# ArjunTeh/AdjointNonlinearRayTracing

Measured on AMD Instinct MI355X. Metric: ray-steps/sec (fwd+adjoint), 256^3 RIF grid, 1M rays x 512 steps, higher is better.
Workload: dtype f32

## Files before the change

adjointnonlinearraytracing_amd/_lib.py:

```python
from __future__ import annotations

import ctypes as C
import os
from typing import Optional

_HERE = os.path.dirname(os.path.abspath(__file__))
LIB_PATH = os.environ.get("DRRT_HIP_LIB") or os.path.join(_HERE, "libdrrt_hip.so")

FLAG_NONE = 0
FLAG_SORT_RAYS = 1
FLAG_CORRECTED_H = 2
FLAG_NO_ZERO = 4
FLAG_DIRECT_ATOMICS = 8
FLAG_DEBUG_COUNTERS = 16
FLAG_PAIR_GRID = 64
FLAG_PAIR_REUSE = 128
FLAG_QUAD_GRID, FLAG_QUAD_REUSE = FLAG_PAIR_GRID, FLAG_PAIR_REUSE
FLAG_Q16_POS_ONLY = 0x200000
FLAG_STATIC_WINDOW = 0x400000
FLAG_CHORD_KEY = 0x800000
FLAG_RING_WINDOW = 0x1000000
FLAG_DISPATCH_IN_ORDER = 0x2000000
FLAG_RING_SPARSE, FLAG_RING_GENERAL, FLAG_RING_DIRECT = 0x4000000, 0x8000000, 0x10000000
ADAM_MASK_BOUNDARY, ADAM_CLAMP_MIN = 1, 2

ERR_RES_MISMATCH, ERR_BAD_RES, ERR_ARG, ERR_HIP = -1, -2, -3, -4


class Stats(C.Structure):
    _fields_ = [("ray_steps", C.c_ulonglong), ("n_failed", C.c_ulonglong),
                ("iters", C.c_uint), ("reserved", C.c_uint)]


STATS_BYTES = C.sizeof(Stats)

_vp, _f, _sz, _u, _ll, _i = C.c_void_p, C.c_float, C.c_size_t, C.c_uint, C.c_longlong, C.c_int
_d = C.c_double
_tail = [_vp, _vp, _sz, _u, _vp]

SIGNATURES = {
    "drrt_workspace_bytes": (_sz, [_sz, _u]),
    "drrt_workspace_bytes_grid": (_sz, [_sz, _ll, _u]),
    "drrt_last_error": (C.c_char_p, []),
    "drrt_version": (C.c_char_p, []),
    "drrt_trace_f32": (_i, [_vp, _ll, _vp, _sz, _vp, _vp, _f, _f, _vp, _vp] + _tail),
    "drrt_trace_f16io": (_i, [_vp, _ll, _vp, _sz, _vp, _vp, _f, _f, _vp, _vp] + _tail),
# ... 19 lines not shown
    "drrt_backtrace_sdf_rays_f32": (_i, [_vp, _vp, _ll, _vp, _sz, _vp, _vp, _vp, _vp, _f, _f, _vp, _vp] + _tail),
    "drrt_sensor_splat_f32": (_i, [_sz, _vp, _vp, _vp, _f, _vp, _vp, _vp, _vp, _i, _f, _vp, _u, _vp]),
    "drrt_sensor_splat_bwd_f32": (_i, [_sz, _vp, _vp, _vp, _f, _vp, _vp, _vp, _vp, _i, _f, _vp, _vp, _vp, _vp]),
    "drrt_sensor_far_splat_f32": (_i, [_sz, _vp, _vp, _f, _vp, _vp, _i, _f, _vp, _u, _vp]),
    "drrt_sensor_far_splat_bwd_f32": (_i, [_sz, _vp, _vp, _f, _vp, _vp, _i, _f, _vp, _vp, _vp, _vp]),
    "drrt_sensor_tex_get_f32": (_i, [_sz, _vp, _vp, _vp, _vp, _vp, _vp, _vp, _i, _f, _i, _vp, _vp]),
    "drrt_sensor_tex_get_bwd_f32": (_i, [_sz, _vp, _vp, _vp, _vp, _vp, _vp, _vp, _i, _f, _i, _vp, _vp, _vp, _vp]),
    "drrt_sensor_splat_dframe_f32": (_i, [_sz, _vp, _vp, _vp, _f, _vp, _i, _f, _vp, _u, _vp]),
    "drrt_sensor_splat_dframe_bwd_f32": (_i, [_sz, _vp, _vp, _vp, _f, _vp, _i, _f, _vp, _vp, _vp, _vp]),
    "drrt_sensor_far_splat_dframe_f32": (_i, [_sz, _vp, _vp, _f, _vp, _i, _f, _vp, _u, _vp]),
    "drrt_sensor_far_splat_dframe_bwd_f32": (_i, [_sz, _vp, _vp, _f, _vp, _i, _f, _vp, _vp, _vp, _vp]),
    "drrt_sensor_tex_get_dframe_f32": (_i, [_sz, _vp, _vp, _vp, _vp, _i, _f, _i, _vp, _vp]),
    "drrt_sensor_tex_get_dframe_bwd_f32": (_i, [_sz, _vp, _vp, _vp, _vp, _i, _f, _i, _vp, _vp, _vp, _vp]),
    "drrt_rays_to_plane_f32": (_i, [_sz, _vp, _vp, _vp, _vp, _i, _vp, _vp]),
    "drrt_rays_to_plane_bwd_f32": (_i, [_sz, _vp, _vp, _vp, _vp, _i, _vp, _vp, _vp, _vp]),
    "drrt_upres_volume_f32": (_i, [_vp, _vp, _vp, _vp, _vp]),
    "drrt_adam_step_f32": (_i, [_vp, _vp, _vp, _vp, _vp, _d, _d, _d, _d, _d, _d, _d, _u, _vp]),
    "drrt_gen_workspace_bytes": (_sz, [_i, _i, _i, _i]),
    "drrt_gen_rays_f32": (_i, [_i, _vp, _vp, _i, _i, _i, _i, _d, _d, _i, _i, _vp, _d, _vp, _vp, _vp, _vp, _vp, _sz, _vp]),
    "drrt_gen_cone_rays_f32": (_i, [_vp, _vp, _i, _i, _i, _i, _d, _d, _d, _vp, _d, _vp, _vp, _vp, _vp, _vp, _sz, _vp]),
    "drrt_last_order": (_vp, [_vp]),
    "drrt_set_order_hint": (None, [_vp, _sz]),
    "drrt_order_hint_pending": (_sz, []),
    "drrt_last_steps": (_vp, [_vp]),
    "drrt_set_step_hint": (None, [_vp, _sz]),
    "drrt_last_bundle_counters": (_vp, []),
    "drrt_ring_threshold_pct": (_i, []),
    "drrt_ring_long_threshold_permille": (_i, []),
    "drrt_ring_direct_threshold_pct": (_i, []),
    "drrt_profile_begin": (_i, [_i]),
    "drrt_profile_collect": (_i, [_vp, _vp, _i]),
    "drrt_profile_end": (None, []),
}

PROF_NAMES = {1: "trace", 2: "backtrace", 3: "sort", 4: "zero", 5: "quad", 6: "backtrace_rays",
              7: "backtrace_cable_rays", 8: "backtrace_pln_rays", 9: "backtrace_sdf_rays"}

_lib: Optional[C.CDLL] = None


def load() -> C.CDLL:
    global _lib
    if _lib is not None:
        return _lib
    if not os.path.exists(LIB_PATH):
        raise RuntimeError(
# ... 27 lines not shown
```

adjointnonlinearraytracing_amd/csrc/drrt_api.hip:

```cpp
#include "drrt_march.h"

using namespace drrt;

namespace drrt {
size_t sort_workspace_bytes(size_t n);
hipError_t sort_rays_by_entry_voxel(const Vol& V, float h, size_t n, const void* pos, const void* vel, int io_half,
                                    float dir_sign, void* ws, size_t ws_bytes, const uint32_t** perm_out,
                                    hipStream_t stream, bool chord_key);
}

static thread_local char g_err[512] = "";

static int fail(int code, const char* msg) {
  snprintf(g_err, sizeof(g_err), "%s", msg);
  return code;
}
static int fail_hip(hipError_t e, const char* where) {
  snprintf(g_err, sizeof(g_err), "%s: %s", where, hipGetErrorString(e));
  return DRRT_ERR_HIP;
}

namespace drrt { int sensor_fail(int code, const char* msg) { return fail(code, msg); } }

extern "C" const char* drrt_last_error(void) { return g_err; }

static thread_local const uint32_t* g_last_order = nullptr;
static thread_local size_t g_last_order_n = 0;
static thread_local const uint32_t* g_hint_order = nullptr;
static thread_local size_t g_hint_n = 0;

static thread_local const uint32_t* g_last_steps = nullptr;
// ... 4 lines not shown
static inline OrderHint take_hint() {
  OrderHint h{g_hint_order, g_hint_n, g_hint_steps, g_hint_steps_n};
  g_hint_order = nullptr; g_hint_n = 0;
  g_hint_steps = nullptr; g_hint_steps_n = 0;
  return h;
}

extern "C" const uint32_t* drrt_last_order(size_t* n_out) {
  if (n_out) *n_out = g_last_order_n;
  return g_last_order;
}
extern "C" void drrt_set_order_hint(const uint32_t* order, size_t n) { g_hint_order = order; g_hint_n = order ? n : 0; }
extern "C" size_t drrt_order_hint_pending(void) { return g_hint_order ? g_hint_n : (g_hint_steps ? g_hint_steps_n : 0); }
extern "C" const uint32_t* drrt_last_steps(size_t* n_out) {
  if (n_out) *n_out = g_last_steps_n;
  return g_last_steps;
}
extern "C" void drrt_set_step_hint(const uint32_t* steps, size_t n) { g_hint_steps = steps; g_hint_steps_n = steps ? n : 0; }
static thread_local const unsigned* g_last_counters = nullptr;
extern "C" const unsigned* drrt_last_bundle_counters(void) { return g_last_counters; }
extern "C" int drrt_ring_threshold_pct(void) { return DRRT_RING_MIN_NOFIT_PCT; }
extern "C" int drrt_ring_long_threshold_permille(void) { return DRRT_RING_MIN_LONG_PERMILLE; }
extern "C" int drrt_ring_direct_threshold_pct(void) { return DRRT_RING_DIRECT_MAX_PAIR_PCT; }

struct ProfRec { hipEvent_t a, b; int id; };
static ProfRec* g_prof = nullptr;
static int g_prof_cap = 0, g_prof_n = 0;

struct ProfScope {
  int slot; hipStream_t s;
  ProfScope(int id, hipStream_t st) : slot(-1), s(st) {
    if (g_prof && g_prof_n < g_prof_cap) {
      slot = g_prof_n++;
      g_prof[slot].id = id;
      (void)hipEventRecord(g_prof[slot].a, s);
    }
  }
  ~ProfScope() { if (slot >= 0) (void)hipEventRecord(g_prof[slot].b, s); }
};

extern "C" void drrt_profile_end(void) {
  for (int i = 0; i < g_prof_cap; ++i) { (void)hipEventDestroy(g_prof[i].a); (void)hipEventDestroy(g_prof[i].b); }
  delete[] g_prof; g_prof = nullptr; g_prof_cap = g_prof_n = 0;
}

extern "C" int drrt_profile_begin(int capacity) {
// ... 83 lines not shown
  if (nvox >= (1LL << 29)) return fail(DRRT_ERR_ARG, "grid too large (>= 2^29 voxels) for 32-bit byte offsets");
  if (res[0] >= (1 << 24) || res[1] >= (1 << 24) || res[2] >= (1 << 24) || (long long)res[0] * res[1] >= (1 << 24))
    return fail(DRRT_ERR_ARG, "grid extents too large for 24-bit index arithmetic");
  if (!(h > 0.f) || !(h < 3.0e38f)) return fail(DRRT_ERR_ARG, "h and ds must be positive and finite");
  V->data = rif; V->W = res[0]; V->H = res[1]; V->D = res[2];
  vol_finish(*V, h);
  return DRRT_OK;
}

static inline int max3(const int r[3]) { return r[0] > r[1] ? (r[0] > r[2] ? r[0] : r[2]) : (r[1] > r[2] ? r[1] : r[2]); }

static inline int steps_fwd(float h, const int res[3], float ds)  { return (int)(4.0f * h * (float)max3(res) / ds); }
static inline int steps_sdf(float h, const int res[3], float ds)  { return (int)(2.0f * h * (float)max3(res) / ds); }
static inline int steps_adj(float h, const int res[3], float ds)  { return (int)(2.0f * h * (float)max3(res) / ds); }

static int zero_stats(drrt_stats* stats, hipStream_t s) {
  if (!stats) return DRRT_OK;
  hipError_t e = hipMemsetAsync(stats, 0, sizeof(drrt_stats), s);
  return e == hipSuccess ? DRRT_OK : fail_hip(e, "hipMemsetAsync(stats)");
}

static int maybe_sort(const Vol& V, float h, size_t n, const void* pos, const void* vel, float dir_sign,
                      unsigned flags, void* ws, size_t ws_bytes, const uint32_t** perm, hipStream_t s,
                      OrderHint hint, int io_half = 0) {
  *perm = nullptr;
  if (hint.order && hint.n == n) { *perm = hint.order; return DRRT_OK; }
  if (!(flags & DRRT_FLAG_SORT_RAYS) || n < 2) return DRRT_OK;
  if (!ws || ws_bytes < sort_workspace_bytes(n)) return fail(DRRT_ERR_ARG, "workspace too small for DRRT_FLAG_SORT_RAYS");
  ProfScope prof(DRRT_PROF_SORT, s);
  hipError_t e = sort_rays_by_entry_voxel(V, h, n, pos, vel, io_half, dir_sign, ws, ws_bytes, perm, s,
                                          (flags & DRRT_FLAG_CHORD_KEY) != 0);
  if (e == hipSuccess) { g_last_order = *perm; g_last_order_n = n; }
  return e == hipSuccess ? DRRT_OK : fail_hip(e, "sort_rays_by_entry_voxel");
}

#define LAUNCH_CHECK(where)                                              \
  do { hipError_t e_ = hipGetLastError(); if (e_ != hipSuccess) return fail_hip(e_, where); } while (0)

static int private_stats(drrt_stats** stats) {
  constexpr int kMaxDev = 64;
  static drrt_stats* priv[kMaxDev] = {};
  int dev = 0;
  hipError_t e = hipGetDevice(&dev);
  if (e != hipSuccess) return fail_hip(e, "hipGetDevice");
  if (dev < 0 || dev >= kMaxDev) return fail(DRRT_ERR_ARG, "device ordinal out of range; pass a stats block");
  if (!priv[dev]) { e = hipMalloc((void**)&priv[dev], sizeof(drrt_stats)); if (e != hipSuccess) return fail_hip(e, "hipMalloc(stats)"); }
  *stats = priv[dev];
  return DRRT_OK;
}

template <int MODE>
static int run_trace(const float* rif, const float* sdf, long long nvox, const int res[3], size_t n,
                     const void* pos, const void* vel, const float* pln_o, const float* pln_d,
                     float h, float ds, void* xt, void* vt, uint8_t* failmask, drrt_stats* stats,
                     void* ws, size_t ws_bytes, unsigned flags, void* stream, int io_half = 0) {
  const OrderHint hint = take_hint();
  g_err[0] = 0;
  hipStream_t s = (hipStream_t)stream;
  TraceArgs a{};
  int rc = make_vol(rif, nvox, res, h, &a.vol); if (rc) return rc;
  rc = check_steps(h, ds); if (rc) return rc;
  if (n == 0) return zero_stats(stats, s);
  if (!pos || !vel || !xt || !vt) return fail(DRRT_ERR_ARG, "null ray pointer");
  if (MODE == 1 && (!pln_o || !pln_d || !failmask)) return fail(DRRT_ERR_ARG, "null plane/failmask pointer");
  if ((MODE == 1 || MODE == 2) && !stats) { rc = private_stats(&stats); if (rc) return rc; }
  if (MODE == 2 && !sdf) return fail(DRRT_ERR_ARG, "null sdf pointer");
  if (n > 0xffffffffULL) return fail(DRRT_ERR_ARG, "too many rays for uint32 permutation");
  rc = zero_stats(stats, s); if (rc) return rc;
  rc = maybe_sort(a.vol, h, n, pos, vel, 1.f, flags, ws, ws_bytes, &a.perm, s, hint, io_half); if (rc) return rc;
  rc = maybe_pair(a.vol, nvox, n, flags, ws, ws_bytes, s); if (rc) return rc;
  if (MODE == 2) {
    const size_t off = (flags & DRRT_FLAG_SORT_RAYS) ? align_up(sort_workspace_bytes(n), 256) : 0;
    if (!ws || ws_bytes < off + n) return fail(DRRT_ERR_ARG, "workspace too small for trace_sdf (see drrt_workspace_bytes)");
    a.again = (uint8_t*)ws + off;
  }
  g_last_steps = nullptr; g_last_steps_n = 0;
  if (MODE != 2) {
    const size_t off = (flags & DRRT_FLAG_SORT_RAYS) ? align_up(sort_workspace_bytes(n), 256) : 0;
    if (ws && ws_bytes >= off + n * sizeof(uint32_t)) {
      a.steps_out = (uint32_t*)((char*)ws + off);
      g_last_steps = a.steps_out; g_last_steps_n = n;
    }
  }
  a.io_half = io_half;
  a.sdf = sdf; a.pos = pos; a.vel = vel; a.pln_o = pln_o; a.pln_d = pln_d;
  a.xt = xt; a.vt = vt; a.failmask = failmask; a.stats = stats; a.n = n; a.ds = ds;
  a.max_steps = (MODE == 2) ? steps_sdf(h, res, ds) : steps_fwd(h, res, ds);
  a.xcd_order = (a.perm != nullptr && !(flags & DRRT_FLAG_DISPATCH_IN_ORDER)) ? 1 : 0;
  {
    ProfScope prof(DRRT_PROF_TRACE, s);
    launch_trace(MODE, a, s);
  }
// ... 115 lines not shown
  if (n == 0) return zero_stats(stats, s);
  if (!pos || !vel || !target || !xt || !vt || !dist2) return fail(DRRT_ERR_ARG, "null ray pointer");
  if (n > 0xffffffffULL) return fail(DRRT_ERR_ARG, "too many rays for uint32 permutation");
  if (!stats) return fail(DRRT_ERR_ARG, "trace_target needs a stats block (global loop count)");
  const size_t state_bytes = align_up(n * 7 * sizeof(float), 256);
  const size_t sort_bytes = (flags & DRRT_FLAG_SORT_RAYS) ? align_up(sort_workspace_bytes(n), 256) : 0;
  if (!ws || ws_bytes < state_bytes + sort_bytes) return fail(DRRT_ERR_ARG, "workspace too small for trace_target");
  rc = zero_stats(stats, s); if (rc) return rc;
  a.state = (float*)ws;
  rc = maybe_sort(a.vol, h, n, pos, vel, 1.f, flags, (char*)ws + state_bytes, ws_bytes - state_bytes, &a.perm, s,
                  OrderHint{nullptr, 0, nullptr, 0});
  if (rc) return rc;
  a.pos = pos; a.vel = vel; a.target = target; a.xt = xt; a.vt = vt; a.dist2 = dist2;
  a.stats = stats; a.n = n; a.ds = ds; a.max_steps = steps_fwd(h, res, ds);
  rc = maybe_pair(a.vol, nvox, n, flags, ws, ws_bytes, s); if (rc) return rc;
  launch_target(a, s);
  LAUNCH_CHECK("k_target");
  return DRRT_OK;
}

struct ChunkReq { void* state; size_t state_bytes; int it_begin, it_count; int* progress; };

namespace drrt {
__global__ void k_chunk_progress_init(int* p) {
  const int k = threadIdx.x;
  if (k < 20) p[k] = (k == 12 || k == 19) ? 0 : ((((k < 12 ? k : k - 1) / 3) & 1) ? (int)0x80000000 : 0x7fffffff);
}
}

struct BackPlan {
  bool direct = false;
  bool classify = false;
  bool ring_general = false;
  int ring_sparse = -1;
  bool box = false;
};
static BackPlan plan_backtrace(int mode, unsigned flags, bool chunk, bool dbg, bool classifiable) {
  BackPlan p;
  if (flags & DRRT_FLAG_DIRECT_ATOMICS) { p.direct = true; return p; }
  if ((flags & DRRT_FLAG_RING_WINDOW) && !chunk) {
    if ((flags & DRRT_FLAG_RING_SPARSE) && mode == 0 && !dbg) p.ring_sparse = (flags & DRRT_FLAG_RING_DIRECT) ? 1 : 0;
    else p.ring_general = true;
    return p;
  }
  p.box = true;
  if ((flags & DRRT_FLAG_STATIC_WINDOW) || chunk || !classifiable) return p;
// ... 13 lines not shown
  g_err[0] = 0;
  hipStream_t s = (hipStream_t)stream;
  BackArgs a{};
  int rc = make_vol(rif, nvox, res, h, &a.vol); if (rc) return rc;
  rc = check_steps(h, ds); if (rc) return rc;
  if (!grad) return fail(DRRT_ERR_ARG, "null grad pointer");
  if (MODE == 1 && !sdf) return fail(DRRT_ERR_ARG, "null sdf pointer");
  const unsigned ablation = (flags >> 8) & 0xffu;
  if (ablation > 1u) return fail(DRRT_ERR_ARG, "flags: bits 8..15 must be 0, or 1 (no adjoint launch)");
  const bool first_chunk = ck == nullptr || ck->it_begin == 0;
  if (ck != nullptr) {
    if (ck->it_begin < 0) return fail(DRRT_ERR_ARG, "chunk: it_begin must be >= 0");
    if (flags & DRRT_FLAG_DIRECT_ATOMICS) return fail(DRRT_ERR_ARG, "chunk: not available with DRRT_FLAG_DIRECT_ATOMICS");
    if (!ck->state || ck->state_bytes < drrt_backtrace_chunk_state_bytes(n))
      return fail(DRRT_ERR_ARG, "chunk: state buffer too small (see drrt_backtrace_chunk_state_bytes)");
    if (!first_chunk && (flags & DRRT_FLAG_SORT_RAYS) && !(hint.order && hint.n == n))
      return fail(DRRT_ERR_ARG, "chunk: a resumed chunk needs the visit order of its first chunk (drrt_set_order_hint)");
  }
  if (!(flags & DRRT_FLAG_NO_ZERO) && first_chunk) {
    ProfScope prof(DRRT_PROF_ZERO, s);
    hipError_t e = hipMemsetAsync(grad, 0, (size_t)nvox * sizeof(float), s);
    if (e != hipSuccess) return fail_hip(e, "hipMemsetAsync(grad)");
  }
  if (first_chunk) { rc = zero_stats(stats, s); if (rc) return rc; }
  if (n == 0) return DRRT_OK;
  if (!xt || !vt || !dx || !dv) return fail(DRRT_ERR_ARG, "null ray pointer");
  if (n > 0xffffffffULL) return fail(DRRT_ERR_ARG, "too many rays for uint32 permutation");
  if (ablation == 1u) return DRRT_OK;
  rc = maybe_sort(a.vol, h, n, xt, vt, -1.f, flags, ws, ws_bytes, &a.perm, s, hint, io_half); if (rc) return rc;
  rc = maybe_pair(a.vol, nvox, n, flags, ws, ws_bytes, s); if (rc) return rc;
  a.io_half = io_half;
  a.sdf = sdf; a.xt = xt; a.vt = vt; a.dx = dx; a.dv = dv; a.grad = grad; a.stats = stats;
  a.n = n; a.ds = ds; a.max_steps = steps_adj(h, res, ds);
  if (ck != nullptr) {
    const int left = a.max_steps - ck->it_begin;
    a.max_steps = ck->it_count < 0 ? left : (ck->it_count < left ? ck->it_count : left);
    if (a.max_steps < 0) a.max_steps = 0;
    a.chunk_state = (float*)ck->state; a.chunk_stride = (size_t)adj_grid_for(n) * kAdjBlock;
    a.chunk_resume = first_chunk ? 0 : 1; a.chunk_progress = ck->progress;
    if (ck->progress) { hipLaunchKernelGGL(drrt::k_chunk_progress_init, dim3(1), dim3(64), 0, s, ck->progress); LAUNCH_CHECK("k_chunk_progress_init"); }
  }
  a.grad_scale = (flags & DRRT_FLAG_CORRECTED_H) ? a.vol.inv_h : 1.0f;
  a.fsteps = (hint.steps && hint.steps_n == n) ? hint.steps : nullptr;
  a.xcd_order = (a.perm != nullptr && !(flags & DRRT_FLAG_DISPATCH_IN_ORDER)) ? 1 : 0;
  a.dbg = nullptr;
  if (flags & DRRT_FLAG_DEBUG_COUNTERS) {
    if (!ws || ws_bytes < 512) return fail(DRRT_ERR_ARG, "workspace too small for DRRT_FLAG_DEBUG_COUNTERS");
    a.dbg = (unsigned long long*)((char*)ws + ((ws_bytes - 512) & ~(size_t)7));
    hipError_t e = hipMemsetAsync(a.dbg, 0, 512, s);
    if (e != hipSuccess) return fail_hip(e, "hipMemsetAsync(dbg)");
  }
  const size_t ctr_off = (drrt_workspace_bytes(n, flags) + ((flags & DRRT_FLAG_PAIR_GRID) ? (size_t)nvox * 2 * sizeof(float) : 0) + 7) & ~(size_t)7;
  const bool dbg = a.dbg != nullptr;
  const BackPlan p = plan_backtrace(MODE, flags, ck != nullptr, dbg, a.perm != nullptr && ws && ws_bytes >= ctr_off + 512);
  {
    ProfScope prof(DRRT_PROF_BACKTRACE, s);
    if (p.direct) launch_backtrace_direct(MODE, a, s);
    if (p.classify) {
      a.select = (unsigned*)((char*)ws + ctr_off + 256);
      g_last_counters = a.select;
      hipError_t e = hipMemsetAsync(a.select, 0, 32, s);
      if (e != hipSuccess) return fail_hip(e, "hipMemsetAsync(select)");
      if (p.ring_general) {
        e = hipMemsetAsync((char*)a.select + 20, 1, 1, s);
        if (e != hipSuccess) return fail_hip(e, "hipMemsetAsync(select)");
      }
      launch_bundle_classify(a, s);
    }
    if (p.ring_general) launch_backtrace_ring(MODE, dbg, a, s);
    if (p.ring_sparse >= 0) launch_backtrace_ring_sparse(a, s, p.ring_sparse);
    if (p.box) launch_backtrace_box(MODE, dbg, a, s);
  }
  LAUNCH_CHECK("k_backtrace");
  return DRRT_OK;
}

extern "C" int drrt_backtrace_f32(const float* rif, long long nvox, const int res[3], size_t n,
                                  const float* xt, const float* vt, const float* dx, const float* dv,
                                  float h, float ds, float* grad, drrt_stats* stats, void* ws,
                                  size_t ws_bytes, unsigned flags, void* stream) {
  return run_backtrace<0>(rif, nullptr, nvox, res, n, xt, vt, dx, dv, h, ds, grad, stats, ws, ws_bytes, flags, stream);
}

extern "C" int drrt_backtrace_rays_f32(const float* rif, long long nvox, const int res[3], size_t n,
                                       const float* pos, const float* vel, const float* xt, const float* vt,
                                       const uint32_t* fwd_steps, const float* dx, const float* dv, float h, float ds,
                                       float* dpos, float* dvel, drrt_stats* stats, void* ws, size_t ws_bytes,
                                       unsigned flags, void* stream) {
  const OrderHint hint = take_hint();
  g_err[0] = 0;
  hipStream_t s = (hipStream_t)stream;
// ... 206 lines not shown
```

adjointnonlinearraytracing_amd/csrc/drrt_sort.hip:

```cpp
#include <hip/hip_runtime.h>
#include <hip/hip_fp16.h>
#include <rocprim/device/device_radix_sort.hpp>
#include <stdint.h>

#include "drrt_device.h"

namespace drrt {

constexpr int kKeyBitsPerAxis = 10;
constexpr int kKeyBits = 6 * kKeyBitsPerAxis;

__device__ __forceinline__ float ldr(const Vol& V, const void* p, size_t k, int io, bool is_pos) {
  if (io == 3) return is_pos ? q16_pos_dec(V, ((const uint16_t*)p)[k]) : ((const float*)p)[k];
  if (io == 2) return is_pos ? q16_pos_dec(V, ((const uint16_t*)p)[k]) : q16_vel_dec(((const int16_t*)p)[k]);
  return io ? __half2float(((const __half*)p)[k]) : ((const float*)p)[k];
}

__global__ void __launch_bounds__(256) k_chord_keys(Vol V, size_t n, const void* __restrict__ pos,
                                                    const void* __restrict__ vel, int io_half, float dir_sign,
                                                    uint64_t* __restrict__ keys, uint32_t* __restrict__ idx) {
  size_t i = (size_t)blockIdx.x * 256 + threadIdx.x;
  if (i >= n) return;
  float p[3] = {ldr(V, pos, 3 * i, io_half, true), ldr(V, pos, 3 * i + 1, io_half, true), ldr(V, pos, 3 * i + 2, io_half, true)};
  float d[3] = {dir_sign * ldr(V, vel, 3 * i, io_half, false), dir_sign * ldr(V, vel, 3 * i + 1, io_half, false),
// ... 33 lines not shown
  keys[i] = key;
  idx[i] = (uint32_t)i;
}

constexpr int kDirHalf = 15;
constexpr int kPosBits = 11;
constexpr int kLfKeyBits = 2 * kPosBits + 10;

__device__ __forceinline__ uint32_t hilbert2(uint32_t x, uint32_t y) {
  uint32_t d = 0;
#pragma unroll
  for (int b = kPosBits - 1; b >= 0; --b) {
    const uint32_t s = 1u << b, rx = (x >> b) & 1u, ry = (y >> b) & 1u;
    d += s * s * ((3u * rx) ^ ry);
    if (ry == 0u) {
      if (rx == 1u) { x = s - 1u - x; y = s - 1u - y; }
      const uint32_t t = x; x = y; y = t;
    }
    x &= s - 1u; y &= s - 1u;
  }
  return d;
}

__global__ void __launch_bounds__(256) k_lightfield_keys(Vol V, size_t n, const void* __restrict__ pos,
                                                         const void* __restrict__ vel, int io_half, float dir_sign,
                                                         uint32_t* __restrict__ keys, uint32_t* __restrict__ idx) {
  size_t i = (size_t)blockIdx.x * 256 + threadIdx.x;
  if (i >= n) return;
  const float p[3] = {ldr(V, pos, 3 * i, io_half, true), ldr(V, pos, 3 * i + 1, io_half, true), ldr(V, pos, 3 * i + 2, io_half, true)};
  float d[3] = {dir_sign * ldr(V, vel, 3 * i, io_half, false), dir_sign * ldr(V, vel, 3 * i + 1, io_half, false),
                dir_sign * ldr(V, vel, 3 * i + 2, io_half, false)};
  idx[i] = (uint32_t)i;
  const float len = sqrtf(d[0] * d[0] + d[1] * d[1] + d[2] * d[2]);
  if (!(len > 1e-30f) || !(len < 3.0e38f)) { keys[i] = 0; return; }
  const float il = 1.f / len;
  d[0] *= il; d[1] *= il; d[2] *= il;
  const float l1 = fabsf(d[0]) + fabsf(d[1]) + fabsf(d[2]);
  float ox = d[0] / l1, oy = d[1] / l1;
  if (d[2] < 0.f) {
    const float fx = (1.f - fabsf(oy)) * (ox >= 0.f ? 1.f : -1.f), fy = (1.f - fabsf(ox)) * (oy >= 0.f ? 1.f : -1.f);
    ox = fx; oy = fy;
  }
  int a = (int)rintf(ox * (float)kDirHalf), b = (int)rintf(oy * (float)kDirHalf);
  a = a < -kDirHalf ? -kDirHalf : (a > kDirHalf ? kDirHalf : a);
  b = b < -kDirHalf ? -kDirHalf : (b > kDirHalf ? kDirHalf : b);
  float cx = (float)a / (float)kDirHalf, cy = (float)b / (float)kDirHalf, cz = 1.f - fabsf(cx) - fabsf(cy);
  if (cz < 0.f) {
    const float fx = (1.f - fabsf(cy)) * (cx >= 0.f ? 1.f : -1.f), fy = (1.f - fabsf(cx)) * (cy >= 0.f ? 1.f : -1.f);
    cx = fx; cy = fy;
  }
  const float cl = 1.f / sqrtf(cx * cx + cy * cy + cz * cz);
  const float c[3] = {cx * cl, cy * cl, cz * cl};
  int ax = 0;
  if (fabsf(c[1]) < fabsf(c[ax])) ax = 1;
  if (fabsf(c[2]) < fabsf(c[ax])) ax = 2;
  float t1[3] = {-c[ax] * c[0], -c[ax] * c[1], -c[ax] * c[2]};
  t1[ax] += 1.f;
  const float tl = 1.f / sqrtf(t1[0] * t1[0] + t1[1] * t1[1] + t1[2] * t1[2]);
  t1[0] *= tl; t1[1] *= tl; t1[2] *= tl;
  const float t2[3] = {c[1] * t1[2] - c[2] * t1[1], c[2] * t1[0] - c[0] * t1[2], c[0] * t1[1] - c[1] * t1[0]};
  const float w[3] = {p[0] - 0.5f * V.bx, p[1] - 0.5f * V.by, p[2] - 0.5f * V.bz};
  const float wd = w[0] * d[0] + w[1] * d[1] + w[2] * d[2];
  const float q[3] = {w[0] - wd * d[0], w[1] - wd * d[1], w[2] - wd * d[2]};
  const float ext = fmaxf(V.bx, fmaxf(V.by, V.bz));
  const float sc = ext > 0.f ? 0.5f / ext : 0.f;
  const float u = (q[0] * t1[0] + q[1] * t1[1] + q[2] * t1[2]) * sc + 0.5f;
  const float v = (q[0] * t2[0] + q[1] * t2[1] + q[2] * t2[2]) * sc + 0.5f;
  const float cells = (float)(1 << kPosBits);
  const uint32_t qu = (uint32_t)fminf(fmaxf(u * cells, 0.f), cells - 1.f);
  const uint32_t qv = (uint32_t)fminf(fmaxf(v * cells, 0.f), cells - 1.f);
  const uint32_t cell = (uint32_t)((a + kDirHalf) * (2 * kDirHalf + 1) + (b + kDirHalf));
  keys[i] = (cell << (2 * kPosBits)) | hilbert2(qu, qv);
}

static inline size_t al(size_t v) { return (v + 255) / 256 * 256; }

static size_t radix_temp_bytes(size_t n) {
  size_t t64 = 0, t32 = 0;
  hipError_t e = rocprim::radix_sort_pairs(nullptr, t64, (const uint64_t*)nullptr, (uint64_t*)nullptr,
                                          (const uint32_t*)nullptr, (uint32_t*)nullptr, n, 0u, (unsigned)kKeyBits,
                                          (hipStream_t)0);
  hipError_t e2 = rocprim::radix_sort_pairs(nullptr, t32, (const uint32_t*)nullptr, (uint32_t*)nullptr,
                                           (const uint32_t*)nullptr, (uint32_t*)nullptr, n, 0u, (unsigned)kLfKeyBits,
                                           (hipStream_t)0);
  size_t temp = t64 > t32 ? t64 : t32;
  if (e != hipSuccess || e2 != hipSuccess || temp == 0) {
    (void)hipGetLastError();
    temp = n * 32 + (1u << 20);
  }
  return temp;
}

size_t sort_workspace_bytes(size_t n) {
  return 2 * al(n * sizeof(uint64_t)) + 2 * al(n * sizeof(uint32_t)) + al(radix_temp_bytes(n));
}

hipError_t sort_rays_by_entry_voxel(const Vol& V, float h, size_t n, const void* pos, const void* vel, int io_half,
                                    float dir_sign, void* ws, size_t ws_bytes, const uint32_t** perm_out,
                                    hipStream_t stream, bool chord_key) {
  (void)h;
  char* base = (char*)ws;
  const size_t k8 = al(n * sizeof(uint64_t)), k4 = al(n * sizeof(uint32_t));
  uint64_t* keys_in = (uint64_t*)(base);
  uint64_t* keys_out = (uint64_t*)(base + k8);
  uint32_t* idx_in = (uint32_t*)(base + 2 * k8);
  uint32_t* idx_out = (uint32_t*)(base + 2 * k8 + k4);
  void* temp = base + 2 * k8 + 2 * k4;
  size_t temp_bytes = ws_bytes - (2 * k8 + 2 * k4);
  hipError_t e;
  if (chord_key) {
    hipLaunchKernelGGL(k_chord_keys, dim3((unsigned)((n + 255) / 256)), dim3(256), 0, stream, V, n, pos, vel,
                       io_half, dir_sign, keys_in, idx_in);
    e = hipGetLastError();
    if (e != hipSuccess) return e;
    e = rocprim::radix_sort_pairs(temp, temp_bytes, (const uint64_t*)keys_in, keys_out,
                                  (const uint32_t*)idx_in, idx_out, n, 0u, (unsigned)kKeyBits, stream);
  } else {
    hipLaunchKernelGGL(k_lightfield_keys, dim3((unsigned)((n + 255) / 256)), dim3(256), 0, stream, V, n, pos, vel,
                       io_half, dir_sign, (uint32_t*)keys_in, idx_in);
    e = hipGetLastError();
    if (e != hipSuccess) return e;
    e = rocprim::radix_sort_pairs(temp, temp_bytes, (const uint32_t*)keys_in, (uint32_t*)keys_out,
                                  (const uint32_t*)idx_in, idx_out, n, 0u, (unsigned)kLfKeyBits, stream);
  }
  *perm_out = idx_out;
  return e;
}

}
```

adjointnonlinearraytracing_amd/drrt.py:

```python
from __future__ import annotations

import contextlib
import ctypes as C
import dataclasses
import threading
from dataclasses import dataclass
from typing import Dict, Optional, Sequence, Tuple

import torch

from . import _lib


@dataclass
class Options:
    sort_rays: bool = True
    corrected_h: bool = False
    check_failed: bool = True
    direct_atomics: bool = False
    adjoint_window: str = "auto"
    chord_key: bool = False
    pair_grid: object = "auto"

    @property
    def quad_grid(self):
        return self.pair_grid

    @quad_grid.setter
    def quad_grid(self, v):
        self.pair_grid = v


options = Options()

_tls = threading.local()


def _opt() -> Options:
    return getattr(_tls, "options", None) or options


@contextlib.contextmanager
def using(**overrides):
    prev = getattr(_tls, "options", None)
# ... 16 lines not shown
    return (device, torch.cuda.current_stream(device).cuda_stream)


def _flags(adjoint: bool = False) -> int:
    f = 0
    if _opt().sort_rays:
        f |= _lib.FLAG_SORT_RAYS
    if adjoint and _opt().corrected_h:
        f |= _lib.FLAG_CORRECTED_H
    if adjoint and _opt().direct_atomics:
        f |= _lib.FLAG_DIRECT_ATOMICS
    if adjoint and _opt().adjoint_window == "box":
        f |= _lib.FLAG_STATIC_WINDOW
    if adjoint and _opt().adjoint_window == "ring":
        f |= _lib.FLAG_RING_WINDOW
    if adjoint and _opt().adjoint_window == "ring_sparse":
        f |= _lib.FLAG_RING_WINDOW | _lib.FLAG_RING_SPARSE
    if adjoint and _opt().adjoint_window == "ring_direct":
        f |= _lib.FLAG_RING_WINDOW | _lib.FLAG_RING_SPARSE | _lib.FLAG_RING_DIRECT
    if adjoint and _opt().adjoint_window == "ring_general":
        f |= _lib.FLAG_RING_GENERAL
    if _opt().chord_key:
        f |= _lib.FLAG_CHORD_KEY
    return f


def _workspace(n: int, flags: int, device: torch.device, nvox: int = 0) -> torch.Tensor:
    need = int(_lib.load().drrt_workspace_bytes_grid(n, nvox, flags))
    key = _wkey(device)
    ws = _workspaces.get(key)
    if ws is None or ws.numel() < need:
        ws = torch.empty(max(need, 1 << 20), dtype=torch.uint8, device=device)
        _workspaces[key] = ws
        _quad_tokens.pop(key, None)
    if not (flags & _lib.FLAG_PAIR_GRID):
        _quad_tokens.pop(key, None)
    return ws


_quad_tokens: Dict[tuple, tuple] = {}


def _march_workspace(rif_: torch.Tensor, res, n: int, h: float, ds: float, flags: int, device: torch.device,
                     paired: bool = False, adjoint: bool = False):
    q = _opt().pair_grid
    auto = q == "auto"
# ... 594 lines not shown
```

include/drrt_hip.h:

```cpp
#ifndef DRRT_HIP_H
#define DRRT_HIP_H

#include <stddef.h>
#include <stdint.h>

#ifdef __cplusplus
extern "C" {
#endif

#if defined(__GNUC__)
#define DRRT_API __attribute__((visibility("default")))
#else
#define DRRT_API
#endif

#define DRRT_OK                0
#define DRRT_ERR_RES_MISMATCH (-1)
#define DRRT_ERR_BAD_RES      (-2)
#define DRRT_ERR_ARG          (-3)
#define DRRT_ERR_HIP          (-4)

#define DRRT_FLAG_NONE         0u
#define DRRT_FLAG_SORT_RAYS    1u
#define DRRT_FLAG_CORRECTED_H  2u
#define DRRT_FLAG_NO_ZERO      4u
#define DRRT_FLAG_DIRECT_ATOMICS 8u

#define DRRT_FLAG_PAIR_GRID    64u
#define DRRT_FLAG_PAIR_REUSE  128u
#define DRRT_FLAG_QUAD_GRID  DRRT_FLAG_PAIR_GRID
#define DRRT_FLAG_QUAD_REUSE DRRT_FLAG_PAIR_REUSE
#define DRRT_FLAG_Q16_POS_ONLY 0x200000u
#define DRRT_FLAG_CHORD_KEY 0x800000u
#define DRRT_FLAG_RING_WINDOW 0x1000000u
#define DRRT_FLAG_RING_SPARSE  0x4000000u
#define DRRT_FLAG_RING_GENERAL 0x8000000u
#define DRRT_FLAG_RING_DIRECT  0x10000000u
#define DRRT_FLAG_STATIC_WINDOW 0x400000u
#define DRRT_FLAG_DISPATCH_IN_ORDER 0x2000000u
#define DRRT_FLAG_DEBUG_COUNTERS 16u


typedef struct drrt_stats {
  unsigned long long ray_steps;
  unsigned long long n_failed;
  unsigned int       iters;
  unsigned int       reserved;
} drrt_stats;

DRRT_API size_t drrt_workspace_bytes(size_t n, unsigned flags);
DRRT_API size_t drrt_workspace_bytes_grid(size_t n, long long nvox, unsigned flags);

DRRT_API const char* drrt_last_error(void);

DRRT_API const char* drrt_version(void);

DRRT_API const uint32_t* drrt_last_order(size_t* n_out);
DRRT_API void drrt_set_order_hint(const uint32_t* order, size_t n);
DRRT_API size_t drrt_order_hint_pending(void);
DRRT_API const uint32_t* drrt_last_steps(size_t* n_out);
DRRT_API void drrt_set_step_hint(const uint32_t* steps, size_t n);

DRRT_API const unsigned* drrt_last_bundle_counters(void);
DRRT_API int drrt_ring_threshold_pct(void);
DRRT_API int drrt_ring_long_threshold_permille(void);
DRRT_API int drrt_ring_direct_threshold_pct(void);

DRRT_API int drrt_q16_params(const int res[3], float h, float out[3]);
DRRT_API int drrt_q16_encode(const int res[3], float h, size_t n, const float* pos, const float* vel,
                    void* pos_q, void* vel_q, void* stream);
DRRT_API int drrt_q16_decode(const int res[3], float h, size_t n, const void* pos_q, const void* vel_q,
                    float* pos, float* vel, void* stream);
DRRT_API int drrt_trace_q16io(const float* rif, long long nvox, const int res[3], size_t n,
                     const void* pos_q, const void* vel_q, float h, float ds,
                     void* xt_q, void* vt_q,
                     drrt_stats* stats, void* workspace, size_t workspace_bytes,
                     unsigned flags, void* stream);
DRRT_API int drrt_backtrace_q16io(const float* rif, long long nvox, const int res[3], size_t n,
                         const void* xt_q, const void* vt_q, const void* dx_h, const void* dv_h,
                         float h, float ds, float* grad,
                         drrt_stats* stats, void* workspace, size_t workspace_bytes,
// ... 184 lines not shown
```

Measured before the change: 90.02 billion.

## Replace rocprim ray sort with custom fused 8-bit radix sort and merged clears

Result: no change. 89.77 billion (-0.3%).

```diff
diff --git a/adjointnonlinearraytracing_amd/_lib.py b/adjointnonlinearraytracing_amd/_lib.py
--- a/adjointnonlinearraytracing_amd/_lib.py
+++ b/adjointnonlinearraytracing_amd/_lib.py
@@ -22,6 +22,7 @@
 FLAG_RING_WINDOW = 0x1000000
 FLAG_DISPATCH_IN_ORDER = 0x2000000
 FLAG_RING_SPARSE, FLAG_RING_GENERAL, FLAG_RING_DIRECT = 0x4000000, 0x8000000, 0x10000000
+FLAG_SORT_ROCPRIM = 0x20000000
 ADAM_MASK_BOUNDARY, ADAM_CLAMP_MIN = 1, 2
 
 ERR_RES_MISMATCH, ERR_BAD_RES, ERR_ARG, ERR_HIP = -1, -2, -3, -4
@@ -87,6 +88,7 @@
     "drrt_last_order": (_vp, [_vp]),
     "drrt_set_order_hint": (None, [_vp, _sz]),
     "drrt_order_hint_pending": (_sz, []),
+    "drrt_sort_tile_size": (_u, []),
     "drrt_last_steps": (_vp, [_vp]),
     "drrt_set_step_hint": (None, [_vp, _sz]),
     "drrt_last_bundle_counters": (_vp, []),
diff --git a/adjointnonlinearraytracing_amd/csrc/drrt_api.hip b/adjointnonlinearraytracing_amd/csrc/drrt_api.hip
--- a/adjointnonlinearraytracing_amd/csrc/drrt_api.hip
+++ b/adjointnonlinearraytracing_amd/csrc/drrt_api.hip
@@ -6,7 +6,9 @@
 size_t sort_workspace_bytes(size_t n);
 hipError_t sort_rays_by_entry_voxel(const Vol& V, float h, size_t n, const void* pos, const void* vel, int io_half,
                                     float dir_sign, void* ws, size_t ws_bytes, const uint32_t** perm_out,
-                                    hipStream_t stream, bool chord_key);
+                                    hipStream_t stream, bool chord_key, bool force_rocprim, void* zero_stats,
+                                    unsigned zero_stats_words, bool* stats_zeroed);
+unsigned sort_tile_size();
 }
 
 static thread_local char g_err[512] = "";
@@ -57,6 +59,7 @@
 extern "C" int drrt_ring_threshold_pct(void) { return DRRT_RING_MIN_NOFIT_PCT; }
 extern "C" int drrt_ring_long_threshold_permille(void) { return DRRT_RING_MIN_LONG_PERMILLE; }
 extern "C" int drrt_ring_direct_threshold_pct(void) { return DRRT_RING_DIRECT_MAX_PAIR_PCT; }
+extern "C" unsigned drrt_sort_tile_size(void) { return drrt::sort_tile_size(); }
 
 struct ProfRec { hipEvent_t a, b; int id; };
 static ProfRec* g_prof = nullptr;
@@ -186,14 +189,16 @@
 
 static int maybe_sort(const Vol& V, float h, size_t n, const void* pos, const void* vel, float dir_sign,
                       unsigned flags, void* ws, size_t ws_bytes, const uint32_t** perm, hipStream_t s,
-                      OrderHint hint, int io_half = 0) {
+                      OrderHint hint, int io_half = 0, drrt_stats* stats = nullptr, bool* stats_zeroed = nullptr) {
   *perm = nullptr;
+  if (stats_zeroed) *stats_zeroed = false;
   if (hint.order && hint.n == n) { *perm = hint.order; return DRRT_OK; }
   if (!(flags & DRRT_FLAG_SORT_RAYS) || n < 2) return DRRT_OK;
   if (!ws || ws_bytes < sort_workspace_bytes(n)) return fail(DRRT_ERR_ARG, "workspace too small for DRRT_FLAG_SORT_RAYS");
   ProfScope prof(DRRT_PROF_SORT, s);
   hipError_t e = sort_rays_by_entry_voxel(V, h, n, pos, vel, io_half, dir_sign, ws, ws_bytes, perm, s,
-                                          (flags & DRRT_FLAG_CHORD_KEY) != 0);
+                                          (flags & DRRT_FLAG_CHORD_KEY) != 0, (flags & DRRT_FLAG_SORT_ROCPRIM) != 0, stats,
+                                          (unsigned)(sizeof(drrt_stats) / sizeof(uint32_t)), stats_zeroed);
   if (e == hipSuccess) { g_last_order = *perm; g_last_order_n = n; }
   return e == hipSuccess ? DRRT_OK : fail_hip(e, "sort_rays_by_entry_voxel");
 }
@@ -230,8 +235,9 @@
   if ((MODE == 1 || MODE == 2) && !stats) { rc = private_stats(&stats); if (rc) return rc; }
   if (MODE == 2 && !sdf) return fail(DRRT_ERR_ARG, "null sdf pointer");
   if (n > 0xffffffffULL) return fail(DRRT_ERR_ARG, "too many rays for uint32 permutation");
-  rc = zero_stats(stats, s); if (rc) return rc;
-  rc = maybe_sort(a.vol, h, n, pos, vel, 1.f, flags, ws, ws_bytes, &a.perm, s, hint, io_half); if (rc) return rc;
+  bool stats_zeroed = false;
+  rc = maybe_sort(a.vol, h, n, pos, vel, 1.f, flags, ws, ws_bytes, &a.perm, s, hint, io_half, stats, &stats_zeroed); if (rc) return rc;
+  if (!stats_zeroed) { rc = zero_stats(stats, s); if (rc) return rc; }
   rc = maybe_pair(a.vol, nvox, n, flags, ws, ws_bytes, s); if (rc) return rc;
   if (MODE == 2) {
     const size_t off = (flags & DRRT_FLAG_SORT_RAYS) ? align_up(sort_workspace_bytes(n), 256) : 0;
@@ -393,6 +399,13 @@
 struct ChunkReq { void* state; size_t state_bytes; int it_begin, it_count; int* progress; };
 
 namespace drrt {
+struct ClearReq { uint32_t* a; unsigned na; uint32_t* b; unsigned nb; uint32_t* c; unsigned nc; int c_one; };
+__global__ void __launch_bounds__(256) k_clear_counters(ClearReq r) {
+  const unsigned t = threadIdx.x;
+  if (t < r.na) r.a[t] = 0u;
+  if (t < r.nb) r.b[t] = 0u;
+  if (t < r.nc) r.c[t] = ((int)t == r.c_one) ? 1u : 0u;
+}
 __global__ void k_chunk_progress_init(int* p) {
   const int k = threadIdx.x;
   if (k < 20) p[k] = (k == 12 || k == 19) ? 0 : ((((k < 12 ? k : k - 1) / 3) & 1) ? (int)0x80000000 : 0x7fffffff);
@@ -452,11 +465,11 @@
     hipError_t e = hipMemsetAsync(grad, 0, (size_t)nvox * sizeof(float), s);
     if (e != hipSuccess) return fail_hip(e, "hipMemsetAsync(grad)");
   }
-  if (first_chunk) { rc = zero_stats(stats, s); if (rc) return rc; }
-  if (n == 0) return DRRT_OK;
+  drrt_stats* const stats_to_zero = first_chunk ? stats : nullptr;
+  if (n == 0) return zero_stats(stats_to_zero, s);
   if (!xt || !vt || !dx || !dv) return fail(DRRT_ERR_ARG, "null ray pointer");
   if (n > 0xffffffffULL) return fail(DRRT_ERR_ARG, "too many rays for uint32 permutation");
-  if (ablation == 1u) return DRRT_OK;
+  if (ablation == 1u) return zero_stats(stats_to_zero, s);
   rc = maybe_sort(a.vol, h, n, xt, vt, -1.f, flags, ws, ws_bytes, &a.perm, s, hint, io_half); if (rc) return rc;
   rc = maybe_pair(a.vol, nvox, n, flags, ws, ws_bytes, s); if (rc) return rc;
   a.io_half = io_half;
@@ -477,26 +490,28 @@
   if (flags & DRRT_FLAG_DEBUG_COUNTERS) {
     if (!ws || ws_bytes < 512) return fail(DRRT_ERR_ARG, "workspace too small for DRRT_FLAG_DEBUG_COUNTERS");
     a.dbg = (unsigned long long*)((char*)ws + ((ws_bytes - 512) & ~(size_t)7));
-    hipError_t e = hipMemsetAsync(a.dbg, 0, 512, s);
-    if (e != hipSuccess) return fail_hip(e, "hipMemsetAsync(dbg)");
   }
   const size_t ctr_off = (drrt_workspace_bytes(n, flags) + ((flags & DRRT_FLAG_PAIR_GRID) ? (size_t)nvox * 2 * sizeof(float) : 0) + 7) & ~(size_t)7;
   const bool dbg = a.dbg != nullptr;
   const BackPlan p = plan_backtrace(MODE, flags, ck != nullptr, dbg, a.perm != nullptr && ws && ws_bytes >= ctr_off + 512);
   {
     ProfScope prof(DRRT_PROF_BACKTRACE, s);
-    if (p.direct) launch_backtrace_direct(MODE, a, s);
+    drrt::ClearReq clr{};
+    clr.c_one = -1;
+    if (stats_to_zero) { clr.a = (uint32_t*)stats_to_zero; clr.na = (unsigned)(sizeof(drrt_stats) / sizeof(uint32_t)); }
+    if (a.dbg) { clr.b = (uint32_t*)a.dbg; clr.nb = 128; }
     if (p.classify) {
       a.select = (unsigned*)((char*)ws + ctr_off + 256);
       g_last_counters = a.select;
-      hipError_t e = hipMemsetAsync(a.select, 0, 32, s);
-      if (e != hipSuccess) return fail_hip(e, "hipMemsetAsync(select)");
-      if (p.ring_general) {
-        e = hipMemsetAsync((char*)a.select + 20, 1, 1, s);
-        if (e != hipSuccess) return fail_hip(e, "hipMemsetAsync(select)");
-      }
-      launch_bundle_classify(a, s);
+      clr.c = a.select; clr.nc = 8;
+      if (p.ring_general) clr.c_one = 5;
     }
+    if (clr.na || clr.nb || clr.nc) {
+      hipLaunchKernelGGL(drrt::k_clear_counters, dim3(1), dim3(256), 0, s, clr);
+      LAUNCH_CHECK("k_clear_counters");
+    }
+    if (p.direct) launch_backtrace_direct(MODE, a, s);
+    if (p.classify) launch_bundle_classify(a, s);
     if (p.ring_general) launch_backtrace_ring(MODE, dbg, a, s);
     if (p.ring_sparse >= 0) launch_backtrace_ring_sparse(a, s, p.ring_sparse);
     if (p.box) launch_backtrace_box(MODE, dbg, a, s);
diff --git a/adjointnonlinearraytracing_amd/csrc/drrt_sort.hip b/adjointnonlinearraytracing_amd/csrc/drrt_sort.hip
--- a/adjointnonlinearraytracing_amd/csrc/drrt_sort.hip
+++ b/adjointnonlinearraytracing_amd/csrc/drrt_sort.hip
@@ -79,17 +79,9 @@
   return d;
 }
 
-__global__ void __launch_bounds__(256) k_lightfield_keys(Vol V, size_t n, const void* __restrict__ pos,
-                                                         const void* __restrict__ vel, int io_half, float dir_sign,
-                                                         uint32_t* __restrict__ keys, uint32_t* __restrict__ idx) {
-  size_t i = (size_t)blockIdx.x * 256 + threadIdx.x;
-  if (i >= n) return;
-  const float p[3] = {ldr(V, pos, 3 * i, io_half, true), ldr(V, pos, 3 * i + 1, io_half, true), ldr(V, pos, 3 * i + 2, io_half, true)};
-  float d[3] = {dir_sign * ldr(V, vel, 3 * i, io_half, false), dir_sign * ldr(V, vel, 3 * i + 1, io_half, false),
-                dir_sign * ldr(V, vel, 3 * i + 2, io_half, false)};
-  idx[i] = (uint32_t)i;
+__device__ __forceinline__ uint32_t lightfield_key(const Vol& V, const float p[3], float d[3]) {
   const float len = sqrtf(d[0] * d[0] + d[1] * d[1] + d[2] * d[2]);
-  if (!(len > 1e-30f) || !(len < 3.0e38f)) { keys[i] = 0; return; }
+  if (!(len > 1e-30f) || !(len < 3.0e38f)) return 0u;
   const float il = 1.f / len;
   d[0] *= il; d[1] *= il; d[2] *= il;
   const float l1 = fabsf(d[0]) + fabsf(d[1]) + fabsf(d[2]);
@@ -127,8 +119,240 @@
   const uint32_t qu = (uint32_t)fminf(fmaxf(u * cells, 0.f), cells - 1.f);
   const uint32_t qv = (uint32_t)fminf(fmaxf(v * cells, 0.f), cells - 1.f);
   const uint32_t cell = (uint32_t)((a + kDirHalf) * (2 * kDirHalf + 1) + (b + kDirHalf));
-  keys[i] = (cell << (2 * kPosBits)) | hilbert2(qu, qv);
-}
+  return (cell << (2 * kPosBits)) | hilbert2(qu, qv);
+}
+
+__global__ void __launch_bounds__(256) k_lightfield_keys(Vol V, size_t n, const void* __restrict__ pos,
+                                                         const void* __restrict__ vel, int io_half, float dir_sign,
+                                                         uint32_t* __restrict__ keys, uint32_t* __restrict__ idx) {
+  size_t i = (size_t)blockIdx.x * 256 + threadIdx.x;
+  if (i >= n) return;
+  const float p[3] = {ldr(V, pos, 3 * i, io_half, true), ldr(V, pos, 3 * i + 1, io_half, true), ldr(V, pos, 3 * i + 2, io_half, true)};
+  float d[3] = {dir_sign * ldr(V, vel, 3 * i, io_half, false), dir_sign * ldr(V, vel, 3 * i + 1, io_half, false),
+                dir_sign * ldr(V, vel, 3 * i + 2, io_half, false)};
+  idx[i] = (uint32_t)i;
+  keys[i] = lightfield_key(V, p, d);
+}
+
+constexpr unsigned kSortTile = 8192;
+constexpr unsigned kSortItems = kSortTile / 256;
+constexpr unsigned kKeyTile = 2048;
+constexpr unsigned kKeyItems = kKeyTile / 256;
+constexpr size_t kOwnSortMaxN = 4194304;
+constexpr unsigned kSortHistWords = 4 * 256, kSortCurWords = 64;
+
+static inline unsigned sort_tiles(size_t n) { return (unsigned)((n + kSortTile - 1) / kSortTile); }
+static inline size_t own_sort_meta_words(size_t n) { return kSortHistWords + kSortCurWords + (size_t)sort_tiles(n) * 256; }
+
+__global__ void __launch_bounds__(256) k_sort_clear(uint32_t* __restrict__ meta, unsigned words, uint32_t* __restrict__ stats,
+                                                    unsigned stats_words) {
+  const unsigned i = blockIdx.x * 256u + threadIdx.x;
+  if (i < words) meta[i] = 0u;
+  if (blockIdx.x == 0 && threadIdx.x < stats_words) stats[threadIdx.x] = 0u;
+}
+
+__device__ __forceinline__ void lds_hist_add(uint32_t* h, uint32_t dig, bool valid) {
+  const uint32_t first = (uint32_t)__builtin_amdgcn_readfirstlane((int)dig);
+  if (__all(valid && dig == first)) {
+    if ((threadIdx.x & 63u) == 0u) atomicAdd(&h[first], 64u);
+  } else if (valid) {
+    atomicAdd(&h[dig], 1u);
+  }
+}
+
+__global__ void __launch_bounds__(256) k_lf_keys_hist(Vol V, unsigned n, const void* __restrict__ pos,
+                                                      const void* __restrict__ vel, int io_half, float dir_sign,
+                                                      uint32_t* __restrict__ keys, uint32_t* __restrict__ idx,
+                                                      uint32_t* __restrict__ hist, uint32_t* __restrict__ count0) {
+  __shared__ uint32_t lh[4 * 256];
+  const unsigned tid = threadIdx.x;
+#pragma unroll
+  for (int q = 0; q < 4; ++q) lh[q * 256 + tid] = 0u;
+  __syncthreads();
+  const unsigned base = blockIdx.x * kKeyTile + tid;
+  float p[kKeyItems][3], d[kKeyItems][3];
+#pragma unroll
+  for (unsigned j = 0; j < kKeyItems; ++j) {
+    const unsigned i = base + j * 256u;
+    const size_t k = 3 * (size_t)(i < n ? i : n - 1u);
+#pragma unroll
+    for (int a = 0; a < 3; ++a) {
+      p[j][a] = ldr(V, pos, k + a, io_half, true);
+      d[j][a] = dir_sign * ldr(V, vel, k + a, io_half, false);
+    }
+  }
+#pragma unroll
+  for (unsigned j = 0; j < kKeyItems; ++j) {
+    const unsigned i = base + j * 256u;
+    const bool valid = i < n;
+    const uint32_t key = lightfield_key(V, p[j], d[j]);
+    if (valid) { keys[i] = key; idx[i] = i; }
+#pragma unroll
+    for (int q = 0; q < 4; ++q) lds_hist_add(lh + q * 256, (key >> (8 * q)) & 255u, valid);
+  }
+  __syncthreads();
+#pragma unroll
+  for (int q = 0; q < 4; ++q) {
+    const uint32_t v = lh[q * 256 + tid];
+    if (v) atomicAdd(&hist[q * 256 + tid], v);
+  }
+  const uint32_t v0 = lh[tid];
+  if (v0) atomicAdd(&count0[(blockIdx.x / (kSortTile / kKeyTile)) * 256u + tid], v0);
+}
+
+__device__ __forceinline__ bool sort_pass_constant(const uint32_t* __restrict__ hist, int pass, unsigned n, uint32_t* flag) {
+  if (threadIdx.x == 0) *flag = 0u;
+  __syncthreads();
+  if (hist[pass * 256 + threadIdx.x] == n) *flag = 1u;
+  __syncthreads();
+  return *flag != 0u;
+}
+
+__global__ void __launch_bounds__(256) k_sort_count(unsigned n, int pass, const uint32_t* __restrict__ hist,
+                                                    const uint32_t* __restrict__ cur, const uint32_t* __restrict__ keysA,
+                                                    const uint32_t* __restrict__ keysB, uint32_t* __restrict__ table) {
+  __shared__ uint32_t lh[256];
+  __shared__ uint32_t flag;
+  const unsigned tid = threadIdx.x;
+  if (sort_pass_constant(hist, pass, n, &flag)) return;
+  const uint32_t* __restrict__ in = cur[pass] ? keysB : keysA;
+  lh[tid] = 0u;
+  __syncthreads();
+  const unsigned base = blockIdx.x * kSortTile + tid;
+  uint32_t k[kSortItems];
+#pragma unroll
+  for (unsigned j = 0; j < kSortItems; ++j) {
+    const unsigned i = base + j * 256u;
+    k[j] = i < n ? in[i] : 0u;
+  }
+#pragma unroll
+  for (unsigned j = 0; j < kSortItems; ++j) lds_hist_add(lh, (k[j] >> (8 * pass)) & 255u, base + j * 256u < n);
+  __syncthreads();
+  table[blockIdx.x * 256u + tid] = lh[tid];
+}
+
+__global__ void __launch_bounds__(256) k_sort_scatter(unsigned n, int pass, const uint32_t* __restrict__ hist,
+                                                      uint32_t* __restrict__ cur, const uint32_t* __restrict__ table,
+                                                      uint32_t* __restrict__ keysA, uint32_t* __restrict__ idxA,
+                                                      uint32_t* __restrict__ keysB, uint32_t* __restrict__ idxB,
+                                                      uint32_t* __restrict__ perm) {
+  __shared__ uint32_t wcnt[4 * 256];
+  __shared__ uint32_t part[4 * 256];
+  __shared__ uint32_t scan[2][256];
+  __shared__ uint32_t constant[4];
+  const unsigned tid = threadIdx.x, lane = tid & 63u, wave = tid >> 6, tile = blockIdx.x;
+  if (tid < 4) constant[tid] = 0u;
+  __syncthreads();
+#pragma unroll
+  for (int q = 0; q < 4; ++q)
+    if (hist[q * 256 + tid] == n) constant[q] = 1u;
+  __syncthreads();
+  const uint32_t src = cur[pass];
+  bool later = false, earlier = false;
+  for (int q = 0; q < 4; ++q) {
+    if (q > pass && !constant[q]) later = true;
+    if (q < pass && !constant[q]) earlier = true;
+  }
+  if (constant[pass]) {
+    if (tile == 0 && tid == 0) cur[pass + 1] = src;
+    if (pass == 3 && !earlier) {
+      for (unsigned j = 0; j < kSortItems; ++j) {
+        const unsigned i = tile * kSortTile + j * 256u + tid;
+        if (i < n) perm[i] = i;
+      }
+    }
+    return;
+  }
+  if (tile == 0 && tid == 0) cur[pass + 1] = src ^ 1u;
+  const uint32_t* __restrict__ kin = src ? keysB : keysA;
+  const uint32_t* __restrict__ iin = src ? idxB : idxA;
+  uint32_t* __restrict__ kout = src ? keysA : keysB;
+  uint32_t* __restrict__ iout = later ? (src ? idxA : idxB) : perm;
+
+  const unsigned first = tile * kSortTile + wave * (kSortTile / 4) + lane;
+  uint32_t key[kSortItems];
+#pragma unroll
+  for (unsigned r = 0; r < kSortItems; ++r) {
+    const unsigned i = first + r * 64u;
+    key[r] = i < n ? kin[i] : 0u;
+  }
+
+  const uint32_t h = hist[pass * 256 + tid];
+  scan[0][tid] = h;
+  __syncthreads();
+  int sb = 0;
+#pragma unroll
+  for (unsigned o = 1; o < 256; o <<= 1) {
+    const uint32_t v = scan[sb][tid] + (tid >= o ? scan[sb][tid - o] : 0u);
+    scan[sb ^ 1][tid] = v;
+    sb ^= 1;
+    __syncthreads();
+  }
+  uint32_t start = scan[sb][tid] - h;
+
+  {
+    uint4 acc = make_uint4(0u, 0u, 0u, 0u);
+#pragma unroll 8
+    for (unsigned t = wave; t < tile; t += 4) {
+      const uint4 v = ((const uint4*)(table + (size_t)t * 256u))[lane];
+      acc.x += v.x; acc.y += v.y; acc.z += v.z; acc.w += v.w;
+    }
+    ((uint4*)(part + wave * 256u))[lane] = acc;
+  }
+#pragma unroll
+  for (int w = 0; w < 4; ++w) wcnt[w * 256 + tid] = 0u;
+  __syncthreads();
+  start += part[tid] + part[256 + tid] + part[512 + tid] + part[768 + tid];
+
+  volatile uint32_t* wc = wcnt + wave * 256u;
+  uint32_t rank[kSortItems];
+#pragma unroll
+  for (unsigned r = 0; r < kSortItems; ++r) {
+    const bool valid = first + r * 64u < n;
+    const uint32_t dig = (key[r] >> (8 * pass)) & 255u;
+    unsigned long long m = __ballot(valid);
+#pragma unroll
+    for (int b = 0; b < 8; ++b) {
+      const bool bit = (dig >> b) & 1u;
+      const unsigned long long bal = __ballot(bit);
+      m &= bit ? bal : ~bal;
+    }
+    const uint32_t below = __builtin_amdgcn_mbcnt_hi((uint32_t)(m >> 32), __builtin_amdgcn_mbcnt_lo((uint32_t)m, 0u));
+    const uint32_t prev = wc[dig];
+    rank[r] = prev + below;
+    __builtin_amdgcn_wave_barrier();
+    if (valid && below == 0u) wc[dig] = prev + (uint32_t)__popcll(m);
+    __builtin_amdgcn_wave_barrier();
+  }
+  __syncthreads();
+  {
+    uint32_t run = start;
+#pragma unroll
+    for (int w = 0; w < 4; ++w) {
+      const uint32_t c = wcnt[w * 256 + tid];
+      wcnt[w * 256 + tid] = run;
+      run += c;
+    }
+  }
+  __syncthreads();
+
+  uint32_t id[kSortItems];
+#pragma unroll
+  for (unsigned r = 0; r < kSortItems; ++r) {
+    const unsigned i = first + r * 64u;
+    id[r] = i < n ? iin[i] : 0u;
+  }
+#pragma unroll
+  for (unsigned r = 0; r < kSortItems; ++r) {
+    const uint32_t dig = (key[r] >> (8 * pass)) & 255u;
+    const uint32_t at = wcnt[wave * 256u + dig] + rank[r];
+    if (first + r * 64u < n && at < n) {
+      if (later) kout[at] = key[r];
+      iout[at] = id[r];
+    }
+  }
+}
+
 
 static inline size_t al(size_t v) { return (v + 255) / 256 * 256; }
 
@@ -148,14 +372,28 @@
   return temp;
 }
 
+unsigned sort_tile_size() { return kSortTile; }
+
 size_t sort_workspace_bytes(size_t n) {
-  return 2 * al(n * sizeof(uint64_t)) + 2 * al(n * sizeof(uint32_t)) + al(radix_temp_bytes(n));
-}
+  size_t temp = radix_temp_bytes(n);
+  const size_t own = n <= kOwnSortMaxN ? own_sort_meta_words(n) * sizeof(uint32_t) : 0;
+  if (own > temp) temp = own;
+  return 2 * al(n * sizeof(uint64_t)) + 2 * al(n * sizeof(uint32_t)) + al(temp);
+}
+
+#define SORT_LAUNCH(kernel, grid, ...)                                                        \
+  do {                                                                                        \
+    hipLaunchKernelGGL(kernel, dim3(grid), dim3(256), 0, stream, __VA_ARGS__);                \
+    hipError_t e_ = hipGetLastError();                                                        \
+    if (e_ != hipSuccess) return e_;                                                          \
+  } while (0)
 
 hipError_t sort_rays_by_entry_voxel(const Vol& V, float h, size_t n, const void* pos, const void* vel, int io_half,
                                     float dir_sign, void* ws, size_t ws_bytes, const uint32_t** perm_out,
-                                    hipStream_t stream, bool chord_key) {
+                                    hipStream_t stream, bool chord_key, bool force_rocprim, void* zero_stats,
+                                    unsigned zero_stats_words, bool* stats_zeroed) {
   (void)h;
+  if (stats_zeroed) *stats_zeroed = false;
   char* base = (char*)ws;
   const size_t k8 = al(n * sizeof(uint64_t)), k4 = al(n * sizeof(uint32_t));
   uint64_t* keys_in = (uint64_t*)(base);
@@ -172,13 +410,29 @@
     if (e != hipSuccess) return e;
     e = rocprim::radix_sort_pairs(temp, temp_bytes, (const uint64_t*)keys_in, keys_out,
                                   (const uint32_t*)idx_in, idx_out, n, 0u, (unsigned)kKeyBits, stream);
-  } else {
+  } else if (force_rocprim || n > kOwnSortMaxN || n < 2) {
     hipLaunchKernelGGL(k_lightfield_keys, dim3((unsigned)((n + 255) / 256)), dim3(256), 0, stream, V, n, pos, vel,
                        io_half, dir_sign, (uint32_t*)keys_in, idx_in);
     e = hipGetLastError();
     if (e != hipSuccess) return e;
     e = rocprim::radix_sort_pairs(temp, temp_bytes, (const uint32_t*)keys_in, (uint32_t*)keys_out,
                                   (const uint32_t*)idx_in, idx_out, n, 0u, (unsigned)kLfKeyBits, stream);
+  } else {
+    const unsigned nn = (unsigned)n, tiles = sort_tiles(n), words = (unsigned)own_sort_meta_words(n);
+    uint32_t* keysA = (uint32_t*)keys_in;
+    uint32_t* idxB = keysA + n;
+    uint32_t* keysB = (uint32_t*)keys_out;
+    uint32_t* hist = (uint32_t*)temp;
+    uint32_t* cur = hist + kSortHistWords;
+    uint32_t* table = cur + kSortCurWords;
+    SORT_LAUNCH(k_sort_clear, (words + 255) / 256, hist, words, (uint32_t*)zero_stats, zero_stats ? zero_stats_words : 0u);
+    if (stats_zeroed) *stats_zeroed = zero_stats != nullptr;
+    SORT_LAUNCH(k_lf_keys_hist, (nn + kKeyTile - 1) / kKeyTile, V, nn, pos, vel, io_half, dir_sign, keysA, idx_in, hist, table);
+    for (int pass = 0; pass < 4; ++pass) {
+      if (pass > 0) SORT_LAUNCH(k_sort_count, tiles, nn, pass, hist, cur, keysA, keysB, table);
+      SORT_LAUNCH(k_sort_scatter, tiles, nn, pass, hist, cur, table, keysA, idx_in, keysB, idxB, idx_out);
+    }
+    e = hipSuccess;
   }
   *perm_out = idx_out;
   return e;
diff --git a/adjointnonlinearraytracing_amd/drrt.py b/adjointnonlinearraytracing_amd/drrt.py
--- a/adjointnonlinearraytracing_amd/drrt.py
+++ b/adjointnonlinearraytracing_amd/drrt.py
@@ -20,6 +20,7 @@
     direct_atomics: bool = False
     adjoint_window: str = "auto"
     chord_key: bool = False
+    sort_rocprim: bool = False
     pair_grid: object = "auto"
 
     @property
@@ -82,6 +83,8 @@
         f |= _lib.FLAG_RING_GENERAL
     if _opt().chord_key:
         f |= _lib.FLAG_CHORD_KEY
+    if _opt().sort_rocprim:
+        f |= _lib.FLAG_SORT_ROCPRIM
     return f
 
 
diff --git a/include/drrt_hip.h b/include/drrt_hip.h
--- a/include/drrt_hip.h
+++ b/include/drrt_hip.h
@@ -32,6 +32,7 @@
 #define DRRT_FLAG_QUAD_REUSE DRRT_FLAG_PAIR_REUSE
 #define DRRT_FLAG_Q16_POS_ONLY 0x200000u
 #define DRRT_FLAG_CHORD_KEY 0x800000u
+#define DRRT_FLAG_SORT_ROCPRIM 0x20000000u
 #define DRRT_FLAG_RING_WINDOW 0x1000000u
 #define DRRT_FLAG_RING_SPARSE  0x4000000u
 #define DRRT_FLAG_RING_GENERAL 0x8000000u
@@ -57,6 +58,7 @@
 
 DRRT_API const uint32_t* drrt_last_order(size_t* n_out);
 DRRT_API void drrt_set_order_hint(const uint32_t* order, size_t n);
+DRRT_API unsigned drrt_sort_tile_size(void);
 DRRT_API size_t drrt_order_hint_pending(void);
 DRRT_API const uint32_t* drrt_last_steps(size_t* n_out);
 DRRT_API void drrt_set_step_hint(const uint32_t* steps, size_t n);
```
